# beehive-lab/GPULlama3.java

Measured on NVIDIA H100. Metric: decode_tokens_per_s, higher is better.
Workload: dtype q8_0xq8_0->int32, f32 accumulate

## Files before the change

### gpullama3.java_b200/csrc/decode_persistent.cuh

```cuda
#pragma once
#include "decode_kernels.cuh"
#include "seqsum2.cuh"
#include "stream_matvec.cuh"

#define PD_WARPS 16
#define PD_CT (PD_WARPS * 32)
#define PD_THREADS (PD_CT + 32)
#define PD_MAX_STAGES 32
#define PD_TIMEOUT_NS 4000000000ull
#define PD_STAMPS 20

enum { PD_S_QKV = 0, PD_S_ATT = 1, PD_S_WO = 2, PD_S_GU = 3, PD_S_W2 = 4, PD_S_LM = 5, PD_S_ARG = 6, PD_S_SLOTS = 8,
       PD_S_TICK = 8, PD_S_LMTICK = 9, PD_S_ERR = 10, PD_S_WORDS = 16 };

struct PdLayer {
    TileMat qkv, wo, gu, w2;
    const float *attn_norm, *ffn_norm, *q_norm, *k_norm;
    const float *qkv_bias;
    float *kc, *vc;
};

struct PdArgs {
    const PdLayer *layers;
    int n_layers;
// ... 360 lines not shown
        pd_bar_sync();
        if (tid == 0) {
            float bv = -INFINITY;
            int bi = 0x7fffffff;
            for (int k = 0; k < PD_WARPS * 4; k++) {
                const float v = hvals[k];
                const int ix = cand_i[k];
                if (v > bv || (v == bv && ix < bi)) { bv = v; bi = ix; }
            }
            a.part_val[blockIdx.x] = bv;
            a.part_idx[blockIdx.x] = bi;
        }
    }
}

__device__ __forceinline__ float4 pd_ldcg128(const float *p) {
    float4 v;
    asm volatile("ld.global.cg.v4.f32 {%0,%1,%2,%3}, [%4];" : "=f"(v.x), "=f"(v.y), "=f"(v.z), "=f"(v.w) : "l"(p));
    return v;
}

__device__ __noinline__ float pd_seqsum(const float *sq, int n, int S, unsigned char *smem, const PdSmem &L, int tid) {
    SeqSum2Scratch scratch = seqsum2_carve(smem + L.off_seq, PD_CT);
    return block_seqsum_exact_v2_t<PD_CT>(sq, n, scratch, tid, PdConsumerSync(), S);
}

__device__ __forceinline__ void pd_prefetch_w(const float *w, float *sbuf, int dim, int tid) {
    const int n4 = dim >> 2;
    for (int i4 = tid; i4 < n4; i4 += PD_CT)
        asm volatile("cp.async.cg.shared.global [%0], [%1], 16;" ::"r"(smem_u32(sbuf + 4 * i4)), "l"(w + 4 * i4) : "memory");
    asm volatile("cp.async.commit_group;" ::: "memory");
}

template <int U>
__device__ __noinline__ void pd_norm_u(const PdArgs &a, const float *wbuf, bool from_emb, int token, unsigned char *smem, const PdSmem &L, int tid, int stamp_layer) {
    const int dim = a.dim, n4 = dim >> 2;
    float *sq = reinterpret_cast<float *>(smem + L.off_nbuf);
    float *misc = reinterpret_cast<float *>(smem + L.off_misc);
    const int E = (dim + PD_CT - 1) / PD_CT, S = seqsum2_stride(E);
    float4 xv[U];
#pragma unroll
    for (int u = 0; u < U; u++) {
        const int i4 = u * PD_CT + tid;
        xv[u] = make_float4(0.f, 0.f, 0.f, 0.f);
        if (i4 < n4) {
            if (from_emb) {
                xv[u] = make_float4(pd_emb_get(a.emb, token, 4 * i4, a.emb_scale), pd_emb_get(a.emb, token, 4 * i4 + 1, a.emb_scale),
                                    pd_emb_get(a.emb, token, 4 * i4 + 2, a.emb_scale), pd_emb_get(a.emb, token, 4 * i4 + 3, a.emb_scale));
            } else xv[u] = pd_ldcg128(a.x + 4 * i4);
        }
    }
    for (int i = dim + tid; i < PD_CT * E; i += PD_CT) sq[(i / E) * S + (i % E)] = 0.0f;
#pragma unroll
    for (int u = 0; u < U; u++) {
        const int i4 = u * PD_CT + tid;
        if (i4 < n4) {
            const int i = 4 * i4;
            const float4 q = make_float4(__fmul_rn(xv[u].x, xv[u].x), __fmul_rn(xv[u].y, xv[u].y), __fmul_rn(xv[u].z, xv[u].z), __fmul_rn(xv[u].w, xv[u].w));
            if ((E & 3) == 0) *reinterpret_cast<float4 *>(sq + (i / E) * S + (i % E)) = q;
            else {
                sq[(i / E) * S + (i % E)] = q.x; sq[((i + 1) / E) * S + ((i + 1) % E)] = q.y;
                sq[((i + 2) / E) * S + ((i + 2) % E)] = q.z; sq[((i + 3) / E) * S + ((i + 3) % E)] = q.w;
            }
        }
    }
    pd_bar_sync();
    if (stamp_layer >= 0) pd_stamp(a, stamp_layer, 10, tid);
    float ss = pd_seqsum(sq, dim, S, smem, L, tid);
    if (stamp_layer >= 0) pd_stamp(a, stamp_layer, 11, tid);
    if (tid == 0) {
        ss = __fdiv_rn(ss, (float)dim);
        ss = __fadd_rn(ss, a.eps);
        misc[20] = (float)(1.0 / sqrt((double)ss));
    }
    asm volatile("cp.async.wait_group 0;" ::: "memory");
    pd_bar_sync();
    ss = misc[20];
    unsigned *sxq = reinterpret_cast<unsigned *>(smem + L.off_xq);
    float *sxs = reinterpret_cast<float *>(smem + L.off_xs);
#pragma unroll
    for (int u = 0; u < U; u++) {
        const int i4 = u * PD_CT + tid;
        if (u * PD_CT < n4) {
            float v0 = 0.f, v1 = 0.f, v2 = 0.f, v3 = 0.f;
            if (i4 < n4) {
                const float4 wv = *reinterpret_cast<const float4 *>(wbuf + 4 * i4);
                v0 = __fmul_rn(wv.x, __fmul_rn(ss, xv[u].x)); v1 = __fmul_rn(wv.y, __fmul_rn(ss, xv[u].y));
                v2 = __fmul_rn(wv.z, __fmul_rn(ss, xv[u].z)); v3 = __fmul_rn(wv.w, __fmul_rn(ss, xv[u].w));
            }
            float amax = fmaxf(fmaxf(fabsf(v0), fabsf(v1)), fmaxf(fabsf(v2), fabsf(v3)));
            amax = fmaxf(amax, __shfl_xor_sync(0xffffffffu, amax, 1));
            amax = fmaxf(amax, __shfl_xor_sync(0xffffffffu, amax, 2));
            amax = fmaxf(amax, __shfl_xor_sync(0xffffffffu, amax, 4));
            const float qs = __fdiv_rn(amax, 127.0f);
            const float ascale = __half2float(__float2half_rn(qs));
            const float ainv = qs != 0.0f ? __fdiv_rn(1.0f, qs) : 0.0f;
            const float s0 = __fmul_rn(v0, ainv), s1 = __fmul_rn(v1, ainv), s2 = __fmul_rn(v2, ainv), s3 = __fmul_rn(v3, ainv);
            const int q0 = __float2int_rz(__fadd_rn(s0, copysignf(0.5f, s0))), q1 = __float2int_rz(__fadd_rn(s1, copysignf(0.5f, s1)));
            const int q2 = __float2int_rz(__fadd_rn(s2, copysignf(0.5f, s2))), q3 = __float2int_rz(__fadd_rn(s3, copysignf(0.5f, s3)));
            if (i4 < n4) {
                sxq[i4] = (unsigned)(q0 & 0xff) | ((unsigned)(q1 & 0xff) << 8) | ((unsigned)(q2 & 0xff) << 16) | ((unsigned)(q3 & 0xff) << 24);
                if ((tid & 7) == 0) sxs[i4 >> 3] = ascale;
            }
        }
    }
    pd_bar_sync();
}

__device__ __forceinline__ void pd_norm_to_smem(const PdArgs &a, const float *wbuf, bool from_emb, int token, unsigned char *smem, const PdSmem &L, int tid, int stamp_layer = -1) {
    const int U = ((a.dim >> 2) + PD_CT - 1) / PD_CT;
    if (U <= 1) pd_norm_u<1>(a, wbuf, from_emb, token, smem, L, tid, stamp_layer);
    else if (U == 2) pd_norm_u<2>(a, wbuf, from_emb, token, smem, L, tid, stamp_layer);
    else pd_norm_u<4>(a, wbuf, from_emb, token, smem, L, tid, stamp_layer);
}

__device__ __noinline__ void pd_load_act(const int8_t *q, const float *s, int cols, unsigned char *smem, const PdSmem &L, int tid) {
    int4 *sxq = reinterpret_cast<int4 *>(smem + L.off_xq);
    float *sxs = reinterpret_cast<float *>(smem + L.off_xs);
    const int4 *src = reinterpret_cast<const int4 *>(q);
    const int n16 = cols >> 4, nb = cols >> 5;
    for (int c0 = 0; c0 < n16; c0 += 4 * PD_CT) {
// ... 358 lines not shown
```

### gpullama3.java_b200/csrc/plan.cu

```cuda
#include "../../include/b200llama.h"
#include "decode_kernels.cuh"
#include "prefill.cuh"
#include "stream_matvec.cuh"
#include "stream_matvec_f16.cuh"
#include "kquant.cuh"
#include "decode_persistent.cuh"
#include "sampler.cuh"
#include "decode_batch.cuh"
#include "moe.cuh"

#include <math.h>
#include <stdarg.h>
#include <stdio.h>
#include <stdlib.h>
#include <string.h>

#include <chrono>
#include <string>
#include <thread>
#include <utility>
#include <vector>

namespace {

// ... 29 lines not shown
struct b200_plan {
    b200_config cfg{};
    Uploader up;
    int device = 0;
    int wtype = 0;
    int qd = 0, kvd = 0;
    int prefill_batch = 0;
    cudaStream_t stream = nullptr;
    std::vector<void *> allocs;
    int64_t bytes = 0;
    std::string err;

    DevMat emb{}, out{};
    TileMat tout{};
    bool use_stream = false, use_pdl = false;
    int kflags = 0;
    size_t kq_off = 0;
    bool use_f16_stream = false;
    bool f16_copies = false;
    int n_sms = 148;
    unsigned *blk_cnt = nullptr;
    float *part_val = nullptr;
    int *part_idx = nullptr;
    float *out_norm = nullptr;
    std::vector<LayerW> layers;
    float *rope_cr = nullptr, *rope_ci = nullptr;

    float *x = nullptr, *xb = nullptr, *qkv = nullptr, *hb = nullptr, *hb2 = nullptr, *logits = nullptr;
    int8_t *xq = nullptr, *hq = nullptr;
    float *xs = nullptr, *hs = nullptr;
// ... 454 lines not shown
int launch_stream(b200_plan *p, const TileMat &W, const int8_t *xq, const float *xs, float *out, int8_t *hq, float *hs, bool argmax = false,
                  TraceBuf tr = TraceBuf{nullptr, 0, 0}, int wait_slot = -1, unsigned wait_op = 0, int out_slot = -1, unsigned out_op = 0,
                  int row_base = 0) {
    SmvSmem L = smv_layout(W.cols, W.seg, SMV_SMEM_BUDGET_MAX);
    SmvArgs a;
    a.W = W; a.xq = xq; a.xs = xs; a.out = out; a.hq = hq; a.hs = hs; a.blk_cnt = p->blk_cnt;
    a.oscale = out_scale(p, MODE == SMV_RESID, &W == &p->tout);
    a.part_val = argmax ? p->part_val : nullptr;
    a.part_idx = argmax ? p->part_idx : nullptr;
    a.tr = tr;
    a.tp = p->tp;
    a.wait_slot = wait_slot; a.wait_op = wait_op; a.out_slot = out_slot; a.out_op = out_op; a.row_base = row_base;
    return launch_k(p, p->use_pdl, k_stream_matvec_q8<MODE>, dim3(p->n_sms), dim3(SMV_THREADS), L.total, a, L);
}

bool stream_shape_ok(int rows, int cols) {
    if (rows % 4 || cols % 32) return false;
    int nseg = smv_pick_nseg(cols);
    if (!nseg) return false;
    return smv_layout(cols, cols / nseg, SMV_SMEM_BUDGET_MAX).stages >= 3;
}

bool gateup_fits(int hidden, int n_sms) {
    return 2 * ((hidden / 2) / n_sms + 1) <= SMV_HVALS;
}

size_t att_smem_bytes(int head_size, int ctx, bool scratch) { return (size_t)(3 * head_size + (scratch ? 0 : ctx)) * 4; }

int enqueue_moe_ffn(b200_plan *p, int l, TraceBuf tr) {
    const b200_config &c = p->cfg;
// ... 12 lines not shown
    MoeStreamArgs a;
    a.S = L.sgu; a.X = L.xgu; a.bases = L.gu_bases; a.ids = ids; a.weights = w; a.k = k;
    a.xq = p->xq; a.xs = p->xs; a.out = p->hb; a.hq = p->hq; a.hs = p->hs; a.blk_cnt = p->blk_cnt; a.tr = TraceBuf{tr.rec, tr.slot + 2, 11};
    const SmvSmem GL = smv_layout(c.dim, L.sgu.seg, SMV_SMEM_BUDGET_MAX);
    if ((rc = launch_k(p, p->use_pdl, k_moe_gateup, dim3(p->n_sms), dim3(SMV_THREADS), GL.total, a, GL))) return rc;
    a.S = L.sdn; a.X = L.xdn; a.bases = L.dn_bases;
    a.xq = p->hq; a.xs = p->hs; a.out = p->x; a.hq = nullptr; a.hs = nullptr; a.blk_cnt = nullptr; a.tr = TraceBuf{tr.rec, tr.slot + 3, 12};
    return launch_k(p, p->use_pdl, k_moe_down, dim3(p->n_sms), dim3(SMV_THREADS), p->moe_dl.total, a, p->moe_dl);
}

int enqueue_forward(b200_plan *p, bool with_logits, int *launches, bool trace = false) {
    const b200_config &c = p->cfg;
    const bool q8 = p->wtype == B200_GGML_Q8_0;
    const bool st = p->use_stream, pdl = p->use_pdl, sf = p->use_f16_stream;
    const bool tpar = p->tp.n > 1;
    int n = 0;
    auto TR = [&](int id) { return TraceBuf{trace ? p->trace_rec : nullptr, n, id}; };
    const size_t norm_smem = norm_smem_bytes(c.dim);
    int8_t *xq = q8 ? p->xq : nullptr;
    float *xs = q8 ? p->xs : nullptr;
    float *xbf = q8 ? nullptr : p->xb;
    const size_t ctx_kv = (size_t)c.context_length * p->kvd_l;
    const int rank = p->tp.rank;
    auto norm = [&](bool embed, const float *w, int wait_op) {
        auto go = [&](auto kern) {
            return launch_k(p, pdl, kern, dim3(1), dim3(NORM_THREADS), norm_smem, p->x, (const StepState *)p->st, p->emb, p->mup.embedding_scale, w, c.rms_norm_eps, c.dim, xq, xs, xbf, (long long *)nullptr, TR(1), p->tp, wait_op);
        };
        return embed ? go(k_rmsnorm_quant<true>) : go(k_rmsnorm_quant<false>);
    };
    for (int l = 0; l < c.n_layers; l++) {
        LayerW &L = p->layers[l];
        int rc;
        if ((rc = norm(l == 0, L.attn_norm, l == 0 ? -1 : 4 * (l - 1) + 3))) return rc;
        n++;
        if (st) rc = launch_stream<SMV_STORE>(p, L.tqkv, p->xq, p->xs, p->qkv, nullptr, nullptr, false, TR(2));
        else if (q8) rc = launch_matvec_q8<MODE_STORE>(p, L.qkv, p->xq, p->xs, p->qkv);
        else if (sf) rc = launch_stream_f16<SF_STORE>(p, L.qkv, nullptr, p->xb, p->qkv, TR(2));
        else rc = launch_matvec_f16<MODE_STORE>(p, L.qkv, p->xb, p->qkv);
        if (rc) return rc; n++;
        float *kc = p->key_cache + (size_t)l * ctx_kv, *vc = p->value_cache + (size_t)l * ctx_kv;
        {
            const size_t att_smem = att_smem_bytes(c.head_size, c.context_length, p->att_scratch != nullptr);
            auto att = [&](auto kern) {
                return launch_k(p, pdl, kern, dim3(p->nh_l), dim3(ATT_THREADS), att_smem, p->qkv, kc, vc, (const StepState *)p->st,
                                (const float *)p->rope_cr, (const float *)p->rope_ci, p->nh_l, p->nkv_l, p->kflags, (const float *)L.q_norm,
                                (const float *)L.k_norm, (const float *)L.qkv_bias, c.rms_norm_eps, att_score_arg(p), q8 ? p->attq : nullptr, q8 ? p->atts : nullptr, xbf, TR(4),
                                p->tp, (unsigned)(4 * l + 0), rank * p->nh_l, p->att_scratch, c.context_length);
            };
            if (c.head_size == 128) rc = att(k_attention<128>);
            else if (c.head_size == 64) rc = att(k_attention<64>);
            else if (c.head_size == 256) rc = att(k_attention<256>);
            else if (c.head_size == 96) rc = att(k_attention<96>);
            else rc = att(k_attention<32>);
            if (rc) return rc;
            n++;
        }
        if (st) rc = launch_stream<SMV_RESID>(p, L.two, p->attq, p->atts, p->x, nullptr, nullptr, false, TR(5), tpar ? TP_SLOT_ATT : -1, 4 * l + 0, tpar ? TP_SLOT_X : -1, 4 * l + 1, rank * p->dim_l);
        else if (q8) rc = launch_matvec_q8<MODE_RESID>(p, L.wo, p->xq, p->xs, p->x);
        else if (sf) rc = launch_stream_f16<SF_RESID>(p, L.wo, nullptr, p->xb, p->x, TR(5));
        else rc = launch_matvec_f16<MODE_RESID>(p, L.wo, p->xb, p->x);
        if (rc) return rc; n++;
        if (p->is_moe) {
            if ((rc = enqueue_moe_ffn(p, l, TR(1)))) return rc;
            n += 4;
            continue;
        }
        if ((rc = norm(false, L.ffn_norm, 4 * l + 1))) return rc;
        n++;
        if (st) {
            if ((rc = launch_stream<SMV_GATEUP>(p, L.tgu, p->xq, p->xs, p->hb, p->hq, p->hs, false, TR(6), -1, 0, tpar ? TP_SLOT_HQ : -1, 4 * l + 2, rank * p->hid_l))) return rc; n++;
            if ((rc = launch_stream<SMV_RESID>(p, L.tw2, p->hq, p->hs, p->x, nullptr, nullptr, false, TR(7), tpar ? TP_SLOT_HQ : -1, 4 * l + 2, tpar ? TP_SLOT_X : -1, 4 * l + 3, rank * p->dim_l))) return rc; n++;
        } else if (q8) {
            k_gateup_q8<<<c.hidden_dim / 32, 256, q8_smem_bytes(c.dim, 4, 8), p->stream>>>(
                (const int8_t *)L.w1.qs, L.w1.sc, (const int8_t *)L.w3.qs, L.w3.sc, p->xq, p->xs, c.hidden_dim, c.dim, p->hq, p->hs, p->hb);
            CK(cudaGetLastError()); n++;
            if ((rc = launch_matvec_q8<MODE_RESID>(p, L.w2, p->hq, p->hs, p->x))) return rc; n++;
        } else if (sf) {
            if ((rc = launch_stream_f16<SF_GATEUP>(p, L.w1, &L.w3, p->xb, p->hb, TR(6)))) return rc; n++;
            if ((rc = launch_stream_f16<SF_RESID>(p, L.w2, nullptr, p->hb, p->x, TR(7)))) return rc; n++;
        } else {
            if ((rc = launch_matvec_f16<MODE_STORE>(p, L.w1, p->xb, p->hb))) return rc; n++;
            if ((rc = launch_matvec_f16<MODE_STORE>(p, L.w3, p->xb, p->hb2))) return rc; n++;
            k_swiglu<<<(c.hidden_dim + 255) / 256, 256, 0, p->stream>>>(p->hb, p->hb2, c.hidden_dim);
            CK(cudaGetLastError()); n++;
            if ((rc = launch_matvec_f16<MODE_RESID>(p, L.w2, p->hb, p->x))) return rc; n++;
        }
    }
    const int last_x_op = 4 * (c.n_layers - 1) + 3;
    if (with_logits) {
        int rc;
        if ((rc = norm(false, p->out_norm, last_x_op))) return rc;
        n++;
        if (st) rc = launch_stream<SMV_STORE>(p, p->tout, p->xq, p->xs, p->logits, nullptr, nullptr, true, TR(8), -1, 0, -1, 0, rank * p->voc_l);
        else if (q8) rc = launch_matvec_q8<MODE_STORE>(p, p->out, p->xq, p->xs, p->logits);
        else if (sf) rc = launch_stream_f16<SF_STORE>(p, p->out, nullptr, p->xb, p->logits, TR(8), true);
        else rc = launch_matvec_f16<MODE_STORE>(p, p->out, p->xb, p->logits);
        if (rc) return rc; n++;
    }
    {
        int rc;
        if ((rc = launch_k(p, pdl, k_argmax_advance, dim3(1), dim3(1024), (size_t)0, (const float *)p->logits, c.vocab_size, p->st, (const int *)p->seq_tokens, p->out_ids, with_logits ? 1 : 0,
                           (const float *)(st || sf ? p->part_val : nullptr), (const int *)(st || sf ? p->part_idx : nullptr),
                           sf ? sf_grid(p, c.vocab_size, c.dim, false) : p->n_sms, TR(9), p->tp, with_logits ? -1 : last_x_op))) return rc;
        n++;
    }
    if (launches) *launches = n;
    return B200_OK;
}

int pd_prepare(b200_plan *p) {
    const b200_config &c = p->cfg;
// ... 259 lines not shown
    CK(set_max_dyn(k_attention<32>, maxdyn));
    CK(set_max_dyn(k_attention<64>, maxdyn));
    CK(set_max_dyn(k_attention<128>, maxdyn));
    CK(set_max_dyn(k_attention<96>, maxdyn));
    CK(set_max_dyn(k_attention<256>, maxdyn));
    CK(set_max_dyn(k_matvec_q8<1, MODE_STORE>, maxdyn));
    CK(set_max_dyn(k_matvec_q8<2, MODE_STORE>, maxdyn));
    CK(set_max_dyn(k_matvec_q8<4, MODE_STORE>, maxdyn));
    CK(set_max_dyn(k_matvec_q8<1, MODE_RESID>, maxdyn));
    CK(set_max_dyn(k_matvec_q8<2, MODE_RESID>, maxdyn));
    CK(set_max_dyn(k_matvec_q8<4, MODE_RESID>, maxdyn));
    CK(set_max_dyn(k_gateup_q8, maxdyn));
    CK(cudaFuncSetAttribute(k_stream_matvec_q8<SMV_STORE>, cudaFuncAttributeMaxDynamicSharedMemorySize, (int)SMV_SMEM_BUDGET_MAX));
    CK(cudaFuncSetAttribute(k_stream_matvec_q8<SMV_RESID>, cudaFuncAttributeMaxDynamicSharedMemorySize, (int)SMV_SMEM_BUDGET_MAX));
    CK(cudaFuncSetAttribute(k_stream_matvec_q8<SMV_GATEUP>, cudaFuncAttributeMaxDynamicSharedMemorySize, (int)SMV_SMEM_BUDGET_MAX));
    CK(set_max_dyn(k_matvec_f16<MODE_STORE>, maxdyn));
    CK(set_max_dyn(k_matvec_f16<MODE_RESID>, maxdyn));
    CK(set_max_dyn(k_stream_matvec_f16<16, SF_STORE>, maxdyn));
    CK(set_max_dyn(k_stream_matvec_f16<16, SF_RESID>, maxdyn));
    CK(set_max_dyn(k_stream_matvec_f16<16, SF_GATEUP>, maxdyn));
    CK(set_max_dyn(k_stream_matvec_f16<8, SF_STORE>, maxdyn));
    CK(set_max_dyn(k_stream_matvec_f16<8, SF_RESID>, maxdyn));
    CK(set_max_dyn(k_stream_matvec_f16<8, SF_GATEUP>, maxdyn));
    CK(set_max_dyn(k_rmsnorm_quant_batch<true>, maxdyn));
    CK(set_max_dyn(k_rmsnorm_quant_batch<false>, maxdyn));
    CK(set_max_dyn(k_attention_batch<32>, maxdyn));
    CK(set_max_dyn(k_attention_batch<64>, maxdyn));
    CK(set_max_dyn(k_attention_batch<128>, maxdyn));
    CK(set_max_dyn(k_attention_batch<96>, maxdyn));
    CK(set_max_dyn(k_attention_batch<256>, maxdyn));
// ... 124 lines not shown
        const char *e3 = getenv("B200_F16_STREAM");
        p->use_f16_stream = !(e3 && e3[0] == '0') && p->wtype == B200_GGML_F16 && c.tp_size == 1 && sf_layout(p->qd + 2 * p->kvd, c.dim, c.fp16_lanes, false).ok &&
                            sf_layout(c.dim, p->qd, c.fp16_lanes, false).ok && sf_layout(c.hidden_dim, c.dim, c.fp16_lanes, true).ok &&
                            sf_layout(c.dim, c.hidden_dim, c.fp16_lanes, false).ok && sf_layout(c.vocab_size, c.dim, c.fp16_lanes, false).ok;
        if (p->is_moe) {
            const b200_moe_config &m = p->moe;
            const int hs = m.shared_hidden_dim, he = m.expert_hidden_dim;
            const bool cut = stream_shape_ok(2 * hs, c.dim) && stream_shape_ok(c.dim, hs) && stream_shape_ok(2 * he, c.dim) && stream_shape_ok(c.dim, he) &&
                             gateup_fits(p->moe_hv, p->n_sms);
            if (!cut) return fail(p, B200_ERR_UNSUPPORTED, "expert hidden %d / shared hidden %d at dim %d: the Q8_0 stream layout cannot cut these matrices", he, hs, c.dim);
            p->moe_dl = moe_down_layout(p->moe_hv, hs / smv_pick_nseg(hs), he / smv_pick_nseg(he), SMV_SMEM_BUDGET_MAX);
            if (p->moe_dl.stages < 3) return fail(p, B200_ERR_UNSUPPORTED, "the expert down projection leaves fewer than 3 ring stages of shared memory");
            if (!p->use_stream) return fail(p, B200_ERR_UNSUPPORTED, "Qwen2-MoE needs the Q8_0 streaming layout (this plan would use the non-streaming matvecs)");
        }
        p->use_pdl = p->use_stream || p->use_f16_stream;
        if (c.tp_size > 1 && !p->use_stream) return fail(p, B200_ERR_UNSUPPORTED, "tensor parallelism needs the Q8_0 streaming path");
    }
    size_t stage_bytes = (size_t)34 * (8u << 20);
    if (p->use_stream) {
        size_t m1 = (size_t)c.vocab_size * c.dim, m2 = (size_t)2 * c.hidden_dim * c.dim, m3 = (size_t)(p->qd + 2 * p->kvd) * c.dim;
        size_t mx = m1 > m2 ? m1 : m2;
        if (m3 > mx) mx = m3;
        const size_t m4 = (size_t)2 * p->moe.shared_hidden_dim * c.dim;
        if (m4 > mx) mx = m4;
        size_t need = mx / 32 * 34 + 4096;
        if (need > stage_bytes) stage_bytes = need;
    }
    if (any_kq) {
        stage_bytes = (stage_bytes + 255) & ~(size_t)255;
        p->kq_off = stage_bytes;
// ... 854 lines not shown
    const b200_config &c = p->cfg;
    const bool q8 = p->wtype == B200_GGML_Q8_0;
    CK(cudaSetDevice(p->device));
    std::vector<float> save(c.dim);
    CK(cudaStreamSynchronize(p->stream));
    CK(cudaMemcpy(save.data(), p->x, (size_t)c.dim * 4, cudaMemcpyDeviceToHost));
    if (p->use_stream) {
        auto tb = [&](const TileMat &m) -> int64_t { return (int64_t)m.rows * m.cols / 32 * 34; };
        int64_t bytes = 0;
        int launches = 0, rc;
        auto one = [&](int l) -> int {
            LayerW &L = p->layers[l];
            bool keep = p->use_pdl;
            p->use_pdl = false;
            int r;
            switch (which) {
            case 0: bytes = tb(L.tgu); r = launch_stream<SMV_GATEUP>(p, L.tgu, p->xq, p->xs, p->hb, p->hq, p->hs); break;
            case 1: bytes = tb(L.tw2); r = launch_stream<SMV_RESID>(p, L.tw2, p->hq, p->hs, p->x, nullptr, nullptr); break;
            case 2: bytes = tb(L.tqkv); r = launch_stream<SMV_STORE>(p, L.tqkv, p->xq, p->xs, p->qkv, nullptr, nullptr); break;
            case 3: bytes = tb(L.two); r = launch_stream<SMV_RESID>(p, L.two, p->xq, p->xs, p->x, nullptr, nullptr); break;
            default: bytes = tb(p->tout); r = launch_stream<SMV_STORE>(p, p->tout, p->xq, p->xs, p->logits, nullptr, nullptr); break;
            }
            p->use_pdl = keep;
            return r;
        };
        if (which < 0 || which > 4) return fail(p, B200_ERR_BAD_ARG, "unknown kernel id %d", which);
        for (int l = 0; l < c.n_layers; l++) if ((rc = one(l))) return rc;
        CK(cudaEventRecord(p->ev0, p->stream));
        for (int r = 0; r < reps; r++)
            for (int l = 0; l < c.n_layers; l++) { if ((rc = one(l))) return rc; launches++; }
        CK(cudaEventRecord(p->ev1, p->stream));
        CK(cudaStreamSynchronize(p->stream));
        float ms = 0;
        CK(cudaEventElapsedTime(&ms, p->ev0, p->ev1));
        *avg_ms = ms / launches;
        if (algorithmic_bytes) *algorithmic_bytes = bytes;
// ... 410 lines not shown
```

### gpullama3.java_b200/csrc/stream_matvec.cuh

```cuda
#pragma once
#include "common.cuh"

#define SMV_CONSUMER_WARPS 8
#define SMV_THREADS ((SMV_CONSUMER_WARPS + 1) * 32)
#define SMV_MAX_STAGES 16
#define SMV_HVALS 512

enum { SMV_STORE = 0, SMV_RESID = 1, SMV_GATEUP = 2 };

struct TileMat {
    const unsigned char *base;
    int rows, cols;
    int seg, nseg;
    int unit_bytes;
};

__host__ __device__ inline int smv_pick_nseg(int cols) {
    for (int n = 1; n <= 64; n++)
        if (cols % n == 0 && (cols / n) % 32 == 0 && cols / n <= 2560) return n;
    return 0;
}
__host__ __device__ inline int smv_unit_bytes(int seg) { return (seg + seg / 16 + 15) & ~15; }
__host__ __device__ inline int tile_groups(const TileMat &W) { return (W.rows + 3) >> 2; }

// ... 45 lines not shown
        "WAIT_DONE:\n"
        "}\n" ::"r"(bar), "r"(parity)
        : "memory");
}
__device__ __forceinline__ unsigned long long l2_policy_evict_first() {
    unsigned long long pol;
    asm volatile("createpolicy.fractional.L2::evict_first.b64 %0, 1.0;" : "=l"(pol));
    return pol;
}
__device__ __forceinline__ void bulk_g2s_evict_first(unsigned dst, const void *src, unsigned bytes, unsigned bar, unsigned long long pol) {
    asm volatile("cp.async.bulk.shared::cluster.global.mbarrier::complete_tx::bytes.L2::cache_hint [%0], [%1], %2, [%3], %4;" ::"r"(dst), "l"(src),
                 "r"(bytes), "r"(bar), "l"(pol)
                 : "memory");
}
__device__ __forceinline__ void consumer_bar_sync() { asm volatile("bar.sync 1, %0;" ::"n"(SMV_CONSUMER_WARPS * 32) : "memory"); }

__device__ __forceinline__ float ldcg_f32(const float *p) {
    float v;
    asm volatile("ld.global.cg.f32 %0, [%1];" : "=f"(v) : "l"(p));
    return v;
}

__device__ __forceinline__ float swiglu_exact(float g, float u) {
    float s = __fdiv_rn(g, (float)(1.0 + exp((double)(-g))));
    return __fmul_rn(s, u);
}

__device__ __forceinline__ float pd_walk_terms(float acc, const float *t, int nbs) {
    int b = 0;
    if (nbs >= 16) {
// ... 28 lines not shown
    float oscale;
    int8_t *hq;
    float *hs;
    unsigned *blk_cnt;
    float *part_val;
    int *part_idx;
    TraceBuf tr;
    TpCtx tp;
    int wait_slot;
    unsigned wait_op;
    int out_slot;
    unsigned out_op;
    int row_base;
};

template <int MODE>
__global__ void __launch_bounds__(SMV_THREADS, 1) k_stream_matvec_q8(SmvArgs a, SmvSmem L) {
    extern __shared__ __align__(128) unsigned char smem[];
    const int tid = threadIdx.x, lane = tid & 31, warp = tid >> 5;
    const TileMat W = a.W;
    const int S = L.stages;
    const unsigned bar0 = smem_u32(smem + L.off_bar);
    const int ngroups = tile_groups(W);
    const int g0 = (int)(((long long)blockIdx.x * ngroups) / gridDim.x);
    const int g1 = (int)(((long long)(blockIdx.x + 1) * ngroups) / gridDim.x);
    const int nseg = W.nseg;
    const unsigned tile_bytes = 4u * (unsigned)W.unit_bytes;

    volatile unsigned *rel = reinterpret_cast<volatile unsigned *>(smem + L.off_bar + 2 * SMV_MAX_STAGES * 8);
    if (tid == 0) {
        for (int s = 0; s < S; s++) {
            mbar_init(bar0 + 8 * s, 1);
            mbar_init(bar0 + 8 * (SMV_MAX_STAGES + s), 1);
// ... 15 lines not shown
#pragma unroll 1
                    for (int w = 0; w < nw; w++, seq++) {
                        int st = seq % S;
                        unsigned ph = (seq / S) & 1u;
                        mbar_wait(bar0 + 8 * (SMV_MAX_STAGES + st), ph ^ 1u);
                        unsigned full = bar0 + 8 * st;
                        mbar_expect_tx(full, tile_bytes);
                        const unsigned char *src = W.base + ((size_t)(gb + w) * nseg + s) * tile_bytes;
                        bulk_g2s_evict_first(smem_u32(smem + L.off_ring + (size_t)st * L.stage_bytes), src, tile_bytes, full, pol);
                    }
            }
        }
        return;
    }

    pdl_wait();
    trace_mark(a.tr, 2);
    if (a.tp.n > 1 && a.wait_slot >= 0) {
        if (tid == 0) tp_wait(a.tp, a.wait_slot, tp_seq(a.tp, a.wait_op));
        consumer_bar_sync();
    }
    {
        const int nb = W.cols >> 5;
        int4 *sxq = reinterpret_cast<int4 *>(smem + L.off_xq);
        float *sxs = reinterpret_cast<float *>(smem + L.off_xs);
        const int4 *src = reinterpret_cast<const int4 *>(a.xq);
        for (int c = tid; c < W.cols / 16; c += SMV_CONSUMER_WARPS * 32) sxq[c] = __ldcg(src + c);
        for (int b = tid; b < nb; b += SMV_CONSUMER_WARPS * 32) sxs[b] = __ldcg(a.xs + b);
    }
    consumer_bar_sync();

    const int nbs = W.seg >> 5;
    float *terms = reinterpret_cast<float *>(smem + L.off_terms) + (size_t)warp * 4 * L.nbs_pad;
    const unsigned char *sact = smem + L.off_xq;
    const float *sxs = reinterpret_cast<const float *>(smem + L.off_xs);
    const int hsel = (lane >> 2) & 1;

    float *hvals = reinterpret_cast<float *>(smem + L.off_hvals);
    float best = -INFINITY;
    int best_i = 0x7fffffff;

    unsigned seq_base = 0;
    for (int gb = g0; gb < g1; gb += SMV_CONSUMER_WARPS) {
        const int nw = min(SMV_CONSUMER_WARPS, g1 - gb);
        if (warp < nw) {
// ... 117 lines not shown
                    int ix = cand_i[k];
                    if (v > bv || (v == bv && ix < bi)) { bv = v; bi = ix; }
                }
                a.part_val[blockIdx.x] = bv;
                a.part_idx[blockIdx.x] = bi;
            }
        }
    }
    if (a.tp.n > 1 && a.out_slot >= 0) {
        consumer_bar_sync();
        if (tid == 0) tp_cta_done(a.tp, a.out_slot, tp_seq(a.tp, a.out_op), gridDim.x);
    }
    trace_mark(a.tr, 3);
}

struct RepackSrc {
    const unsigned char *raw[3];
    int rows[3];
    int row0[3];
    int gateup;
};

__global__ void k_repack_tiles(RepackSrc src, unsigned char *dst, int rows, int cols, int seg, int nseg, int unit_bytes) {
    const long long unit_id = blockIdx.x;
    const int r = (int)(unit_id % 4);
    const int s = (int)((unit_id / 4) % nseg);
    const long long G = unit_id / (4LL * nseg);
    long long row;
    const unsigned char *raw;
    if (src.gateup) {
// ... 45 lines not shown
```

Before: 220.9.

## Fuse RMSNorm and activation quantization into streaming q8 matvec prologue

Adds a fused kernel variant in which every CTA's consumer warps recompute the RMSNorm and int8 quantization of the residual stream before streaming weight tiles. This replaces the separate norm kernel launch ahead of the QKV, gate/up and logits matvecs. The norm code is factored into a shared templated helper used by both the persistent and streaming kernels. In exchange, each CTA does redundant norm work and the extra norm scratch shrinks the shared-memory ring stages. It is controlled by a new fuse_norm flag.

```diff
diff --git a/gpullama3.java_b200/csrc/decode_persistent.cuh b/gpullama3.java_b200/csrc/decode_persistent.cuh
--- a/gpullama3.java_b200/csrc/decode_persistent.cuh
+++ b/gpullama3.java_b200/csrc/decode_persistent.cuh
@@ -1,5 +1,6 @@
 #pragma once
 #include "decode_kernels.cuh"
+#include "norm_slots.cuh"
 #include "seqsum2.cuh"
 #include "stream_matvec.cuh"
 
@@ -398,12 +399,6 @@
     }
 }
 
-__device__ __forceinline__ float4 pd_ldcg128(const float *p) {
-    float4 v;
-    asm volatile("ld.global.cg.v4.f32 {%0,%1,%2,%3}, [%4];" : "=f"(v.x), "=f"(v.y), "=f"(v.z), "=f"(v.w) : "l"(p));
-    return v;
-}
-
 __device__ __noinline__ float pd_seqsum(const float *sq, int n, int S, unsigned char *smem, const PdSmem &L, int tid) {
     SeqSum2Scratch scratch = seqsum2_carve(smem + L.off_seq, PD_CT);
     return block_seqsum_exact_v2_t<PD_CT>(sq, n, scratch, tid, PdConsumerSync(), S);
@@ -416,79 +411,37 @@
     asm volatile("cp.async.commit_group;" ::: "memory");
 }
 
+struct PdNormOps {
+    const PdArgs &a;
+    const float *wbuf;
+    unsigned char *smem;
+    const PdSmem &L;
+    int tid, stamp_layer;
+    __device__ __forceinline__ void sync() const { pd_bar_sync(); }
+    __device__ __forceinline__ float seqsum(const float *sq, int n, int S) const { return pd_seqsum(sq, n, S, smem, L, tid); }
+    __device__ __forceinline__ float emb(int token, int i) const { return pd_emb_get(a.emb, token, i, a.emb_scale); }
+    __device__ __forceinline__ float4 x4(int i4) const { return ldcg_f32x4(a.x + 4 * i4); }
+    __device__ __forceinline__ void store_x(int, float4) const {}
+    __device__ __forceinline__ float scale(float ss, int dim, float eps) const {
+        float *misc = reinterpret_cast<float *>(smem + L.off_misc);
+        if (tid == 0) {
+            ss = __fdiv_rn(ss, (float)dim);
+            ss = __fadd_rn(ss, eps);
+            misc[20] = (float)(1.0 / sqrt((double)ss));
+        }
+        asm volatile("cp.async.wait_group 0;" ::: "memory");
+        pd_bar_sync();
+        return misc[20];
+    }
+    template <int U> __device__ __forceinline__ float4 w4(const float4 (&)[U], int, int i4) const { return *reinterpret_cast<const float4 *>(wbuf + 4 * i4); }
+    __device__ __forceinline__ void stamp(int k) const { if (stamp_layer >= 0) pd_stamp(a, stamp_layer, k, tid); }
+};
+
 template <int U>
 __device__ __noinline__ void pd_norm_u(const PdArgs &a, const float *wbuf, bool from_emb, int token, unsigned char *smem, const PdSmem &L, int tid, int stamp_layer) {
-    const int dim = a.dim, n4 = dim >> 2;
-    float *sq = reinterpret_cast<float *>(smem + L.off_nbuf);
-    float *misc = reinterpret_cast<float *>(smem + L.off_misc);
-    const int E = (dim + PD_CT - 1) / PD_CT, S = seqsum2_stride(E);
-    float4 xv[U];
-#pragma unroll
-    for (int u = 0; u < U; u++) {
-        const int i4 = u * PD_CT + tid;
-        xv[u] = make_float4(0.f, 0.f, 0.f, 0.f);
-        if (i4 < n4) {
-            if (from_emb) {
-                xv[u] = make_float4(pd_emb_get(a.emb, token, 4 * i4, a.emb_scale), pd_emb_get(a.emb, token, 4 * i4 + 1, a.emb_scale),
-                                    pd_emb_get(a.emb, token, 4 * i4 + 2, a.emb_scale), pd_emb_get(a.emb, token, 4 * i4 + 3, a.emb_scale));
-            } else xv[u] = pd_ldcg128(a.x + 4 * i4);
-        }
-    }
-    for (int i = dim + tid; i < PD_CT * E; i += PD_CT) sq[(i / E) * S + (i % E)] = 0.0f;
-#pragma unroll
-    for (int u = 0; u < U; u++) {
-        const int i4 = u * PD_CT + tid;
-        if (i4 < n4) {
-            const int i = 4 * i4;
-            const float4 q = make_float4(__fmul_rn(xv[u].x, xv[u].x), __fmul_rn(xv[u].y, xv[u].y), __fmul_rn(xv[u].z, xv[u].z), __fmul_rn(xv[u].w, xv[u].w));
-            if ((E & 3) == 0) *reinterpret_cast<float4 *>(sq + (i / E) * S + (i % E)) = q;
-            else {
-                sq[(i / E) * S + (i % E)] = q.x; sq[((i + 1) / E) * S + ((i + 1) % E)] = q.y;
-                sq[((i + 2) / E) * S + ((i + 2) % E)] = q.z; sq[((i + 3) / E) * S + ((i + 3) % E)] = q.w;
-            }
-        }
-    }
-    pd_bar_sync();
-    if (stamp_layer >= 0) pd_stamp(a, stamp_layer, 10, tid);
-    float ss = pd_seqsum(sq, dim, S, smem, L, tid);
-    if (stamp_layer >= 0) pd_stamp(a, stamp_layer, 11, tid);
-    if (tid == 0) {
-        ss = __fdiv_rn(ss, (float)dim);
-        ss = __fadd_rn(ss, a.eps);
-        misc[20] = (float)(1.0 / sqrt((double)ss));
-    }
-    asm volatile("cp.async.wait_group 0;" ::: "memory");
-    pd_bar_sync();
-    ss = misc[20];
-    unsigned *sxq = reinterpret_cast<unsigned *>(smem + L.off_xq);
-    float *sxs = reinterpret_cast<float *>(smem + L.off_xs);
-#pragma unroll
-    for (int u = 0; u < U; u++) {
-        const int i4 = u * PD_CT + tid;
-        if (u * PD_CT < n4) {
-            float v0 = 0.f, v1 = 0.f, v2 = 0.f, v3 = 0.f;
-            if (i4 < n4) {
-                const float4 wv = *reinterpret_cast<const float4 *>(wbuf + 4 * i4);
-                v0 = __fmul_rn(wv.x, __fmul_rn(ss, xv[u].x)); v1 = __fmul_rn(wv.y, __fmul_rn(ss, xv[u].y));
-                v2 = __fmul_rn(wv.z, __fmul_rn(ss, xv[u].z)); v3 = __fmul_rn(wv.w, __fmul_rn(ss, xv[u].w));
-            }
-            float amax = fmaxf(fmaxf(fabsf(v0), fabsf(v1)), fmaxf(fabsf(v2), fabsf(v3)));
-            amax = fmaxf(amax, __shfl_xor_sync(0xffffffffu, amax, 1));
-            amax = fmaxf(amax, __shfl_xor_sync(0xffffffffu, amax, 2));
-            amax = fmaxf(amax, __shfl_xor_sync(0xffffffffu, amax, 4));
-            const float qs = __fdiv_rn(amax, 127.0f);
-            const float ascale = __half2float(__float2half_rn(qs));
-            const float ainv = qs != 0.0f ? __fdiv_rn(1.0f, qs) : 0.0f;
-            const float s0 = __fmul_rn(v0, ainv), s1 = __fmul_rn(v1, ainv), s2 = __fmul_rn(v2, ainv), s3 = __fmul_rn(v3, ainv);
-            const int q0 = __float2int_rz(__fadd_rn(s0, copysignf(0.5f, s0))), q1 = __float2int_rz(__fadd_rn(s1, copysignf(0.5f, s1)));
-            const int q2 = __float2int_rz(__fadd_rn(s2, copysignf(0.5f, s2))), q3 = __float2int_rz(__fadd_rn(s3, copysignf(0.5f, s3)));
-            if (i4 < n4) {
-                sxq[i4] = (unsigned)(q0 & 0xff) | ((unsigned)(q1 & 0xff) << 8) | ((unsigned)(q2 & 0xff) << 16) | ((unsigned)(q3 & 0xff) << 24);
-                if ((tid & 7) == 0) sxs[i4 >> 3] = ascale;
-            }
-        }
-    }
-    pd_bar_sync();
+    const float4 wv[U] = {};
+    norm_quant_slots<PD_CT, U>(PdNormOps{a, wbuf, smem, L, tid, stamp_layer}, from_emb, token, a.dim, a.eps, wv, reinterpret_cast<float *>(smem + L.off_nbuf),
+                               reinterpret_cast<unsigned *>(smem + L.off_xq), reinterpret_cast<float *>(smem + L.off_xs), tid);
 }
 
 __device__ __forceinline__ void pd_norm_to_smem(const PdArgs &a, const float *wbuf, bool from_emb, int token, unsigned char *smem, const PdSmem &L, int tid, int stamp_layer = -1) {
diff --git a/gpullama3.java_b200/csrc/norm_slots.cuh b/gpullama3.java_b200/csrc/norm_slots.cuh
--- /dev/null
+++ b/gpullama3.java_b200/csrc/norm_slots.cuh
@@ -0,0 +1,76 @@
+#pragma once
+#include "common.cuh"
+#include "seqsum2.cuh"
+
+__device__ __forceinline__ float4 ldcg_f32x4(const float *p) {
+    float4 v;
+    asm volatile("ld.global.cg.v4.f32 {%0,%1,%2,%3}, [%4];" : "=f"(v.x), "=f"(v.y), "=f"(v.z), "=f"(v.w) : "l"(p));
+    return v;
+}
+
+__host__ __device__ inline int norm_slots_sq_floats(int dim, int T) { return T * seqsum2_stride((dim + T - 1) / T); }
+
+template <int T, int U, class Ops>
+__device__ __forceinline__ void norm_quant_slots(const Ops &ops, bool from_emb, int token, int dim, float eps, const float4 (&wv)[U], float *sq,
+                                                 unsigned *sxq, float *sxs, int tid) {
+    const int n4 = dim >> 2;
+    const int E = (dim + T - 1) / T, S = seqsum2_stride(E);
+    float4 xv[U];
+#pragma unroll
+    for (int u = 0; u < U; u++) {
+        const int i4 = u * T + tid;
+        xv[u] = make_float4(0.f, 0.f, 0.f, 0.f);
+        if (i4 < n4) {
+            if (from_emb) {
+                xv[u] = make_float4(ops.emb(token, 4 * i4), ops.emb(token, 4 * i4 + 1), ops.emb(token, 4 * i4 + 2), ops.emb(token, 4 * i4 + 3));
+                ops.store_x(i4, xv[u]);
+            } else xv[u] = ops.x4(i4);
+        }
+    }
+    for (int i = dim + tid; i < T * E; i += T) sq[(i / E) * S + (i % E)] = 0.0f;
+#pragma unroll
+    for (int u = 0; u < U; u++) {
+        const int i4 = u * T + tid;
+        if (i4 < n4) {
+            const int i = 4 * i4;
+            const float4 q = make_float4(__fmul_rn(xv[u].x, xv[u].x), __fmul_rn(xv[u].y, xv[u].y), __fmul_rn(xv[u].z, xv[u].z), __fmul_rn(xv[u].w, xv[u].w));
+            if ((E & 3) == 0) *reinterpret_cast<float4 *>(sq + (i / E) * S + (i % E)) = q;
+            else {
+                sq[(i / E) * S + (i % E)] = q.x; sq[((i + 1) / E) * S + ((i + 1) % E)] = q.y;
+                sq[((i + 2) / E) * S + ((i + 2) % E)] = q.z; sq[((i + 3) / E) * S + ((i + 3) % E)] = q.w;
+            }
+        }
+    }
+    ops.sync();
+    ops.stamp(10);
+    float ss = ops.seqsum(sq, dim, S);
+    ops.stamp(11);
+    ss = ops.scale(ss, dim, eps);
+#pragma unroll
+    for (int u = 0; u < U; u++) {
+        const int i4 = u * T + tid;
+        if (u * T < n4) {
+            float v0 = 0.f, v1 = 0.f, v2 = 0.f, v3 = 0.f;
+            if (i4 < n4) {
+                const float4 w = ops.w4(wv, u, i4);
+                v0 = __fmul_rn(w.x, __fmul_rn(ss, xv[u].x)); v1 = __fmul_rn(w.y, __fmul_rn(ss, xv[u].y));
+                v2 = __fmul_rn(w.z, __fmul_rn(ss, xv[u].z)); v3 = __fmul_rn(w.w, __fmul_rn(ss, xv[u].w));
+            }
+            float amax = fmaxf(fmaxf(fabsf(v0), fabsf(v1)), fmaxf(fabsf(v2), fabsf(v3)));
+            amax = fmaxf(amax, __shfl_xor_sync(0xffffffffu, amax, 1));
+            amax = fmaxf(amax, __shfl_xor_sync(0xffffffffu, amax, 2));
+            amax = fmaxf(amax, __shfl_xor_sync(0xffffffffu, amax, 4));
+            const float qs = __fdiv_rn(amax, 127.0f);
+            const float ascale = __half2float(__float2half_rn(qs));
+            const float ainv = qs != 0.0f ? __fdiv_rn(1.0f, qs) : 0.0f;
+            const float s0 = __fmul_rn(v0, ainv), s1 = __fmul_rn(v1, ainv), s2 = __fmul_rn(v2, ainv), s3 = __fmul_rn(v3, ainv);
+            const int q0 = __float2int_rz(__fadd_rn(s0, copysignf(0.5f, s0))), q1 = __float2int_rz(__fadd_rn(s1, copysignf(0.5f, s1)));
+            const int q2 = __float2int_rz(__fadd_rn(s2, copysignf(0.5f, s2))), q3 = __float2int_rz(__fadd_rn(s3, copysignf(0.5f, s3)));
+            if (i4 < n4) {
+                sxq[i4] = (unsigned)(q0 & 0xff) | ((unsigned)(q1 & 0xff) << 8) | ((unsigned)(q2 & 0xff) << 16) | ((unsigned)(q3 & 0xff) << 24);
+                if ((tid & 7) == 0) sxs[i4 >> 3] = ascale;
+            }
+        }
+    }
+    ops.sync();
+}
diff --git a/gpullama3.java_b200/csrc/plan.cu b/gpullama3.java_b200/csrc/plan.cu
--- a/gpullama3.java_b200/csrc/plan.cu
+++ b/gpullama3.java_b200/csrc/plan.cu
@@ -67,6 +67,7 @@
     DevMat emb{}, out{};
     TileMat tout{};
     bool use_stream = false, use_pdl = false;
+    bool fuse_norm = false;
     int kflags = 0;
     size_t kq_off = 0;
     bool use_f16_stream = false;
@@ -551,6 +552,30 @@
     return launch_k(p, p->use_pdl, k_stream_matvec_q8<MODE>, dim3(p->n_sms), dim3(SMV_THREADS), L.total, a, L);
 }
 
+template <int MODE>
+int launch_stream_norm(b200_plan *p, const TileMat &W, const float *w, bool from_emb, float *out, int8_t *hq, float *hs, bool argmax, TraceBuf tr, int row_base = 0) {
+    SmvNormArgs n;
+    const SmvSmem L = smv_layout_norm(W.cols, W.seg, SMV_SMEM_BUDGET_MAX, &n.off_sq, &n.off_seq);
+    n.x = p->x; n.w = w; n.st = p->st; n.emb = p->emb; n.emb_scale = p->mup.embedding_scale; n.eps = p->cfg.rms_norm_eps;
+    n.from_emb = from_emb ? 1 : 0; n.x_out = p->x;
+    SmvArgs a;
+    a.W = W; a.xq = nullptr; a.xs = nullptr; a.out = out; a.hq = hq; a.hs = hs; a.blk_cnt = p->blk_cnt;
+    a.oscale = out_scale(p, false, &W == &p->tout);
+    a.part_val = argmax ? p->part_val : nullptr;
+    a.part_idx = argmax ? p->part_idx : nullptr;
+    a.tr = tr;
+    a.tp = p->tp;
+    a.wait_slot = -1; a.wait_op = 0; a.out_slot = -1; a.out_op = 0; a.row_base = row_base;
+    return launch_k(p, p->use_pdl, k_stream_matvec_q8_norm<MODE>, dim3(p->n_sms), dim3(SMV_THREADS), L.total, a, L, n);
+}
+
+bool norm_fusion_ok(int dim) {
+    const int nseg = smv_pick_nseg(dim);
+    if (!nseg || dim % 32 || dim > 5 * 4 * 256) return false;
+    unsigned a, b;
+    return smv_layout_norm(dim, dim / nseg, SMV_SMEM_BUDGET_MAX, &a, &b).stages >= 3;
+}
+
 bool stream_shape_ok(int rows, int cols) {
     if (rows % 4 || cols % 32) return false;
     int nseg = smv_pick_nseg(cols);
@@ -593,6 +618,7 @@
     const bool q8 = p->wtype == B200_GGML_Q8_0;
     const bool st = p->use_stream, pdl = p->use_pdl, sf = p->use_f16_stream;
     const bool tpar = p->tp.n > 1;
+    const bool fz = p->fuse_norm;
     int n = 0;
     auto TR = [&](int id) { return TraceBuf{trace ? p->trace_rec : nullptr, n, id}; };
     const size_t norm_smem = norm_smem_bytes(c.dim);
@@ -610,12 +636,15 @@
     for (int l = 0; l < c.n_layers; l++) {
         LayerW &L = p->layers[l];
         int rc;
-        if ((rc = norm(l == 0, L.attn_norm, l == 0 ? -1 : 4 * (l - 1) + 3))) return rc;
-        n++;
-        if (st) rc = launch_stream<SMV_STORE>(p, L.tqkv, p->xq, p->xs, p->qkv, nullptr, nullptr, false, TR(2));
-        else if (q8) rc = launch_matvec_q8<MODE_STORE>(p, L.qkv, p->xq, p->xs, p->qkv);
-        else if (sf) rc = launch_stream_f16<SF_STORE>(p, L.qkv, nullptr, p->xb, p->qkv, TR(2));
-        else rc = launch_matvec_f16<MODE_STORE>(p, L.qkv, p->xb, p->qkv);
+        if (fz) rc = launch_stream_norm<SMV_STORE>(p, L.tqkv, L.attn_norm, l == 0, p->qkv, nullptr, nullptr, false, TR(2));
+        else {
+            if ((rc = norm(l == 0, L.attn_norm, l == 0 ? -1 : 4 * (l - 1) + 3))) return rc;
+            n++;
+            if (st) rc = launch_stream<SMV_STORE>(p, L.tqkv, p->xq, p->xs, p->qkv, nullptr, nullptr, false, TR(2));
+            else if (q8) rc = launch_matvec_q8<MODE_STORE>(p, L.qkv, p->xq, p->xs, p->qkv);
+            else if (sf) rc = launch_stream_f16<SF_STORE>(p, L.qkv, nullptr, p->xb, p->qkv, TR(2));
+            else rc = launch_matvec_f16<MODE_STORE>(p, L.qkv, p->xb, p->qkv);
+        }
         if (rc) return rc; n++;
         float *kc = p->key_cache + (size_t)l * ctx_kv, *vc = p->value_cache + (size_t)l * ctx_kv;
         {
@@ -644,10 +673,14 @@
             n += 4;
             continue;
         }
-        if ((rc = norm(false, L.ffn_norm, 4 * l + 1))) return rc;
-        n++;
+        if (!fz) {
+            if ((rc = norm(false, L.ffn_norm, 4 * l + 1))) return rc;
+            n++;
+        }
         if (st) {
-            if ((rc = launch_stream<SMV_GATEUP>(p, L.tgu, p->xq, p->xs, p->hb, p->hq, p->hs, false, TR(6), -1, 0, tpar ? TP_SLOT_HQ : -1, 4 * l + 2, rank * p->hid_l))) return rc; n++;
+            if (fz) rc = launch_stream_norm<SMV_GATEUP>(p, L.tgu, L.ffn_norm, false, p->hb, p->hq, p->hs, false, TR(6));
+            else rc = launch_stream<SMV_GATEUP>(p, L.tgu, p->xq, p->xs, p->hb, p->hq, p->hs, false, TR(6), -1, 0, tpar ? TP_SLOT_HQ : -1, 4 * l + 2, rank * p->hid_l);
+            if (rc) return rc; n++;
             if ((rc = launch_stream<SMV_RESID>(p, L.tw2, p->hq, p->hs, p->x, nullptr, nullptr, false, TR(7), tpar ? TP_SLOT_HQ : -1, 4 * l + 2, tpar ? TP_SLOT_X : -1, 4 * l + 3, rank * p->dim_l))) return rc; n++;
         } else if (q8) {
             k_gateup_q8<<<c.hidden_dim / 32, 256, q8_smem_bytes(c.dim, 4, 8), p->stream>>>(
@@ -668,12 +701,15 @@
     const int last_x_op = 4 * (c.n_layers - 1) + 3;
     if (with_logits) {
         int rc;
-        if ((rc = norm(false, p->out_norm, last_x_op))) return rc;
-        n++;
-        if (st) rc = launch_stream<SMV_STORE>(p, p->tout, p->xq, p->xs, p->logits, nullptr, nullptr, true, TR(8), -1, 0, -1, 0, rank * p->voc_l);
-        else if (q8) rc = launch_matvec_q8<MODE_STORE>(p, p->out, p->xq, p->xs, p->logits);
-        else if (sf) rc = launch_stream_f16<SF_STORE>(p, p->out, nullptr, p->xb, p->logits, TR(8), true);
-        else rc = launch_matvec_f16<MODE_STORE>(p, p->out, p->xb, p->logits);
+        if (fz) rc = launch_stream_norm<SMV_STORE>(p, p->tout, p->out_norm, false, p->logits, nullptr, nullptr, true, TR(8));
+        else {
+            if ((rc = norm(false, p->out_norm, last_x_op))) return rc;
+            n++;
+            if (st) rc = launch_stream<SMV_STORE>(p, p->tout, p->xq, p->xs, p->logits, nullptr, nullptr, true, TR(8), -1, 0, -1, 0, rank * p->voc_l);
+            else if (q8) rc = launch_matvec_q8<MODE_STORE>(p, p->out, p->xq, p->xs, p->logits);
+            else if (sf) rc = launch_stream_f16<SF_STORE>(p, p->out, nullptr, p->xb, p->logits, TR(8), true);
+            else rc = launch_matvec_f16<MODE_STORE>(p, p->out, p->xb, p->logits);
+        }
         if (rc) return rc; n++;
     }
     {
@@ -963,6 +999,8 @@
     CK(cudaFuncSetAttribute(k_stream_matvec_q8<SMV_STORE>, cudaFuncAttributeMaxDynamicSharedMemorySize, (int)SMV_SMEM_BUDGET_MAX));
     CK(cudaFuncSetAttribute(k_stream_matvec_q8<SMV_RESID>, cudaFuncAttributeMaxDynamicSharedMemorySize, (int)SMV_SMEM_BUDGET_MAX));
     CK(cudaFuncSetAttribute(k_stream_matvec_q8<SMV_GATEUP>, cudaFuncAttributeMaxDynamicSharedMemorySize, (int)SMV_SMEM_BUDGET_MAX));
+    CK(cudaFuncSetAttribute(k_stream_matvec_q8_norm<SMV_STORE>, cudaFuncAttributeMaxDynamicSharedMemorySize, (int)SMV_SMEM_BUDGET_MAX));
+    CK(cudaFuncSetAttribute(k_stream_matvec_q8_norm<SMV_GATEUP>, cudaFuncAttributeMaxDynamicSharedMemorySize, (int)SMV_SMEM_BUDGET_MAX));
     CK(set_max_dyn(k_matvec_f16<MODE_STORE>, maxdyn));
     CK(set_max_dyn(k_matvec_f16<MODE_RESID>, maxdyn));
     CK(set_max_dyn(k_stream_matvec_f16<16, SF_STORE>, maxdyn));
@@ -1117,6 +1155,7 @@
             if (!p->use_stream) return fail(p, B200_ERR_UNSUPPORTED, "Qwen2-MoE needs the Q8_0 streaming layout (this plan would use the non-streaming matvecs)");
         }
         p->use_pdl = p->use_stream || p->use_f16_stream;
+        p->fuse_norm = p->use_stream && c.tp_size == 1 && !p->is_moe && norm_fusion_ok(c.dim);
         if (c.tp_size > 1 && !p->use_stream) return fail(p, B200_ERR_UNSUPPORTED, "tensor parallelism needs the Q8_0 streaming path");
     }
     size_t stage_bytes = (size_t)34 * (8u << 20);
@@ -2001,12 +2040,26 @@
             bool keep = p->use_pdl;
             p->use_pdl = false;
             int r;
+            const bool fz = p->fuse_norm;
+            const int64_t nw = fz ? (int64_t)c.dim * 4 : 0;
             switch (which) {
-            case 0: bytes = tb(L.tgu); r = launch_stream<SMV_GATEUP>(p, L.tgu, p->xq, p->xs, p->hb, p->hq, p->hs); break;
+            case 0:
+                bytes = tb(L.tgu) + nw;
+                r = fz ? launch_stream_norm<SMV_GATEUP>(p, L.tgu, L.ffn_norm, false, p->hb, p->hq, p->hs, false, TraceBuf{nullptr, 0, 0})
+                       : launch_stream<SMV_GATEUP>(p, L.tgu, p->xq, p->xs, p->hb, p->hq, p->hs);
+                break;
             case 1: bytes = tb(L.tw2); r = launch_stream<SMV_RESID>(p, L.tw2, p->hq, p->hs, p->x, nullptr, nullptr); break;
-            case 2: bytes = tb(L.tqkv); r = launch_stream<SMV_STORE>(p, L.tqkv, p->xq, p->xs, p->qkv, nullptr, nullptr); break;
+            case 2:
+                bytes = tb(L.tqkv) + nw;
+                r = fz ? launch_stream_norm<SMV_STORE>(p, L.tqkv, L.attn_norm, false, p->qkv, nullptr, nullptr, false, TraceBuf{nullptr, 0, 0})
+                       : launch_stream<SMV_STORE>(p, L.tqkv, p->xq, p->xs, p->qkv, nullptr, nullptr);
+                break;
             case 3: bytes = tb(L.two); r = launch_stream<SMV_RESID>(p, L.two, p->xq, p->xs, p->x, nullptr, nullptr); break;
-            default: bytes = tb(p->tout); r = launch_stream<SMV_STORE>(p, p->tout, p->xq, p->xs, p->logits, nullptr, nullptr); break;
+            default:
+                bytes = tb(p->tout) + nw;
+                r = fz ? launch_stream_norm<SMV_STORE>(p, p->tout, p->out_norm, false, p->logits, nullptr, nullptr, false, TraceBuf{nullptr, 0, 0})
+                       : launch_stream<SMV_STORE>(p, p->tout, p->xq, p->xs, p->logits, nullptr, nullptr);
+                break;
             }
             p->use_pdl = keep;
             return r;
diff --git a/gpullama3.java_b200/csrc/stream_matvec.cuh b/gpullama3.java_b200/csrc/stream_matvec.cuh
--- a/gpullama3.java_b200/csrc/stream_matvec.cuh
+++ b/gpullama3.java_b200/csrc/stream_matvec.cuh
@@ -1,5 +1,7 @@
 #pragma once
 #include "common.cuh"
+#include "decode_kernels.cuh"
+#include "norm_slots.cuh"
 
 #define SMV_CONSUMER_WARPS 8
 #define SMV_THREADS ((SMV_CONSUMER_WARPS + 1) * 32)
@@ -83,6 +85,9 @@
                  : "memory");
 }
 __device__ __forceinline__ void consumer_bar_sync() { asm volatile("bar.sync 1, %0;" ::"n"(SMV_CONSUMER_WARPS * 32) : "memory"); }
+struct SmvConsumerSync {
+    __device__ __forceinline__ void operator()() const { consumer_bar_sync(); }
+};
 
 __device__ __forceinline__ float ldcg_f32(const float *p) {
     float v;
@@ -141,9 +146,79 @@
     int row_base;
 };
 
-template <int MODE>
-__global__ void __launch_bounds__(SMV_THREADS, 1) k_stream_matvec_q8(SmvArgs a, SmvSmem L) {
-    extern __shared__ __align__(128) unsigned char smem[];
+struct SmvNormArgs {
+    const float *x;
+    const float *w;
+    const StepState *st;
+    DevMat emb;
+    float emb_scale, eps;
+    int from_emb;
+    float *x_out;
+    unsigned off_sq, off_seq;
+};
+
+__host__ inline SmvSmem smv_layout_norm(int cols, int seg, size_t budget, unsigned *off_sq, unsigned *off_seq) {
+    SmvSmem L = smv_layout(cols, seg, budget);
+    const size_t sq = (size_t)norm_slots_sq_floats(cols, SMV_CONSUMER_WARPS * 32) * 4;
+    const size_t nb = sq + seqsum2_scratch_bytes(SMV_CONSUMER_WARPS * 32);
+    *off_sq = (unsigned)L.off_terms;
+    *off_seq = (unsigned)(L.off_terms + sq);
+    const size_t dead = L.off_ring - L.off_terms;
+    size_t o = L.off_terms + (nb > dead ? nb : dead);
+    o = (o + 127) & ~(size_t)127;
+    L.off_ring = o;
+    long room = (long)budget - (long)o;
+    int s = room > 0 ? (int)(room / L.stage_bytes) : 0;
+    if (s > SMV_MAX_STAGES) s = SMV_MAX_STAGES;
+    L.stages = s;
+    L.total = o + (size_t)s * L.stage_bytes;
+    return L;
+}
+
+__device__ __noinline__ float smv_seqsum(const float *sq, int n, int S, unsigned char *scratch, int tid) {
+    return block_seqsum_exact_v2_t<SMV_CONSUMER_WARPS * 32>(sq, n, seqsum2_carve(scratch, SMV_CONSUMER_WARPS * 32), tid, SmvConsumerSync(), S);
+}
+
+struct SmvNormOps {
+    const SmvNormArgs &n;
+    unsigned char *smem;
+    int tid;
+    bool write_x;
+    __device__ __forceinline__ void sync() const { consumer_bar_sync(); }
+    __device__ __forceinline__ float seqsum(const float *sq, int cnt, int S) const { return smv_seqsum(sq, cnt, S, smem + n.off_seq, tid); }
+    __device__ __forceinline__ float emb(int token, int i) const { return emb_get(n.emb, token, i, n.emb_scale); }
+    __device__ __forceinline__ float4 x4(int i4) const { return ldcg_f32x4(n.x + 4 * i4); }
+    __device__ __forceinline__ void store_x(int i4, float4 v) const {
+        if (write_x) *reinterpret_cast<float4 *>(n.x_out + 4 * i4) = v;
+    }
+    __device__ __forceinline__ float scale(float ss, int dim, float eps) const {
+        ss = __fdiv_rn(ss, (float)dim);
+        ss = __fadd_rn(ss, eps);
+        return (float)(1.0 / sqrt((double)ss));
+    }
+    template <int U> __device__ __forceinline__ float4 w4(const float4 (&wv)[U], int u, int) const { return wv[u]; }
+    __device__ __forceinline__ void stamp(int) const {}
+};
+
+template <int U>
+__device__ __forceinline__ void smv_norm_prologue(const SmvNormArgs &n, int cols, unsigned char *smem, size_t off_xq, size_t off_xs, int tid, const TraceBuf &tr) {
+    constexpr int T = SMV_CONSUMER_WARPS * 32;
+    const int n4 = cols >> 2;
+    float4 wv[U];
+#pragma unroll
+    for (int u = 0; u < U; u++) {
+        const int i4 = u * T + tid;
+        wv[u] = i4 < n4 ? __ldg(reinterpret_cast<const float4 *>(n.w) + i4) : make_float4(0.f, 0.f, 0.f, 0.f);
+    }
+    pdl_wait();
+    trace_mark(tr, 2);
+    const int token = n.from_emb ? n.st->token : 0;
+    norm_quant_slots<T, U>(SmvNormOps{n, smem, tid, n.from_emb && blockIdx.x == 0}, n.from_emb != 0, token, cols, n.eps, wv,
+                           reinterpret_cast<float *>(smem + n.off_sq), reinterpret_cast<unsigned *>(smem + off_xq), reinterpret_cast<float *>(smem + off_xs), tid);
+}
+
+template <int MODE, bool NORM>
+__device__ __forceinline__ void smv_q8_body(const SmvArgs &a, const SmvSmem &L, const SmvNormArgs &na, unsigned char *smem) {
     const int tid = threadIdx.x, lane = tid & 31, warp = tid >> 5;
     const TileMat W = a.W;
     const int S = L.stages;
@@ -189,21 +264,29 @@
         return;
     }
 
-    pdl_wait();
-    trace_mark(a.tr, 2);
-    if (a.tp.n > 1 && a.wait_slot >= 0) {
-        if (tid == 0) tp_wait(a.tp, a.wait_slot, tp_seq(a.tp, a.wait_op));
+    if (NORM) {
+        const int U = ((W.cols >> 2) + SMV_CONSUMER_WARPS * 32 - 1) / (SMV_CONSUMER_WARPS * 32);
+        if (U <= 1) smv_norm_prologue<1>(na, W.cols, smem, L.off_xq, L.off_xs, tid, a.tr);
+        else if (U == 2) smv_norm_prologue<2>(na, W.cols, smem, L.off_xq, L.off_xs, tid, a.tr);
+        else if (U <= 4) smv_norm_prologue<4>(na, W.cols, smem, L.off_xq, L.off_xs, tid, a.tr);
+        else smv_norm_prologue<5>(na, W.cols, smem, L.off_xq, L.off_xs, tid, a.tr);
+    } else {
+        pdl_wait();
+        trace_mark(a.tr, 2);
+        if (a.tp.n > 1 && a.wait_slot >= 0) {
+            if (tid == 0) tp_wait(a.tp, a.wait_slot, tp_seq(a.tp, a.wait_op));
+            consumer_bar_sync();
+        }
+        {
+            const int nb = W.cols >> 5;
+            int4 *sxq = reinterpret_cast<int4 *>(smem + L.off_xq);
+            float *sxs = reinterpret_cast<float *>(smem + L.off_xs);
+            const int4 *src = reinterpret_cast<const int4 *>(a.xq);
+            for (int c = tid; c < W.cols / 16; c += SMV_CONSUMER_WARPS * 32) sxq[c] = __ldcg(src + c);
+            for (int b = tid; b < nb; b += SMV_CONSUMER_WARPS * 32) sxs[b] = __ldcg(a.xs + b);
+        }
         consumer_bar_sync();
     }
-    {
-        const int nb = W.cols >> 5;
-        int4 *sxq = reinterpret_cast<int4 *>(smem + L.off_xq);
-        float *sxs = reinterpret_cast<float *>(smem + L.off_xs);
-        const int4 *src = reinterpret_cast<const int4 *>(a.xq);
-        for (int c = tid; c < W.cols / 16; c += SMV_CONSUMER_WARPS * 32) sxq[c] = __ldcg(src + c);
-        for (int b = tid; b < nb; b += SMV_CONSUMER_WARPS * 32) sxs[b] = __ldcg(a.xs + b);
-    }
-    consumer_bar_sync();
 
     const int nbs = W.seg >> 5;
     float *terms = reinterpret_cast<float *>(smem + L.off_terms) + (size_t)warp * 4 * L.nbs_pad;
@@ -351,6 +434,19 @@
     trace_mark(a.tr, 3);
 }
 
+template <int MODE>
+__global__ void __launch_bounds__(SMV_THREADS, 1) k_stream_matvec_q8(SmvArgs a, SmvSmem L) {
+    extern __shared__ __align__(128) unsigned char smem[];
+    smv_q8_body<MODE, false>(a, L, SmvNormArgs{}, smem);
+}
+
+template <int MODE>
+__global__ void __maxnreg__(96) k_stream_matvec_q8_norm(SmvArgs a, SmvSmem L, SmvNormArgs n) {
+    static_assert(MODE != SMV_RESID, "a residual matvec consumes an activation, not the residual stream");
+    extern __shared__ __align__(128) unsigned char smem[];
+    smv_q8_body<MODE, true>(a, L, n, smem);
+}
+
 struct RepackSrc {
     const unsigned char *raw[3];
     int rows[3];
```

After: 242.0 (median of 6 runs). 9.5% higher.
